# Healthcare-Robotics/assistive-gym

Measured on AMD Instinct MI355X. Metric: env_steps_per_sec, higher is better.
Workload: dtype f32; 1 GPU; FeedingJaco-v1, 4096 lockstep envs per MI355X, random-policy rollout, 5 simulation steps per env step, 50 PGS sweeps; envs_per_gpu=4096, global_envs=4096, reset_pool=256, reset=pool, parallelism=env-sharded x1, obs_allgather=False

## Files before the change

__graft_entry__.py:

```python
import os
import subprocess
import sys

ROOT = os.path.dirname(os.path.abspath(__file__))
if ROOT not in sys.path:
    sys.path.insert(0, ROOT)


def build():
    from assistive_gym_amd.build import build as build_lib
    build_lib(force=True)
    build_lib(out=os.path.join(ROOT, 'assistive_gym_amd', 'lib', 'variants', 'lvs.so'), extra=('-DAGX_PGS_LV=3',), only=['FEEDING'])
    build_lib(out=os.path.join(ROOT, 'assistive_gym_amd', 'lib', 'variants', 'scan4.so'), extra=('-DAGX_GJK_SCAN_WIDE=0', '-DAGX_GJK_SCAN_ONE=0'), only=['FEEDING'])
    build_lib(out=os.path.join(ROOT, 'assistive_gym_amd', 'lib', 'variants', 'finishgjk.so'), extra=('-DAGX_FINISH_SPILL_GJK',), only=['FEEDING'])
    build_lib(out=os.path.join(ROOT, 'assistive_gym_amd', 'lib', 'variants', 'faceplain.so'), extra=('-DAGX_FACE_PLAIN',), only=['FEEDING', 'FEEDING_M'])
    subprocess.check_call(['make', '-C', os.path.join(ROOT, 'oracle')], stdout=subprocess.DEVNULL)
    if os.path.isdir('/root/reference/assistive_gym/envs/assets'):
        from assistive_gym_amd.model import compiler
        compiler.main()
    import assistive_gym_amd
    from assistive_gym_amd import libagx
    L = libagx.load()
    missing = [e for e in libagx.EXPORTS if not hasattr(L, e)]
    assert not missing, missing


def smoke():
    import numpy as np
    sys.path.insert(0, os.path.join(ROOT, 'tests'))
    from assistive_gym_amd import libagx
    from assistive_gym_amd.blob import ModelBlob
    from assistive_gym_amd.vec_env import build_reset_pool
    from oracle_lib import Oracle
    libagx.check(libagx.load().agx_selftest(0), 'agx_selftest')
    n = 64
# ... 23 lines not shown
```

assistive_gym_amd/csrc/agx_env.h:

```cpp
#pragma once

namespace agx {

AGX_DEV void integrate(Ctx& c, const float* gvel, float dv0, float dv1) {
  float* L = c.lds; const int lane = c.lane, n = c.ndof; const float dt = c.dt;
  L[L_VEL + lane] = gvel[lane] + dv0;
  L[L_VEL + lane + 64] = gvel[lane + 64] + dv1;
  wave_sync();
  if (lane < n) {
    const int d = lane;
    float qd = L[L_VEL + d], q = L[L_ST + c.s_q + d] + dt * qd;
    if (c.hooks && (RBI(c, d, AGX_R_KIND) & 5) == 1 && !FROZEN(c, d)) {
      const float lo = DLO(c, d), hi = DHI(c, d);
      if (q < lo - AGX_LIMIT_EPS) { q = lo; qd = 0.f; } else if (q > hi + AGX_LIMIT_EPS) { q = hi; qd = 0.f; }
    }
    L[L_ST + c.s_qd + d] = qd; L[L_ST + c.s_q + d] = q;
  }
  if (lane < c.nfree) {
    const int b = lane, o = n + 6 * b; float* r = L + L_ST + c.s_free + 13 * b;
    v3 v = ld3(L + L_VEL + o), w = ld3(L + L_VEL + o + 3);
    st3(r + 7, v); st3(r + 10, w); st3(r, ld3(r) + dt * v);
    float wn = sqrtf(dot(w, w)), th = wn * dt; float dq[4];
    if (th > 1e-12f) { float sc = sinf(0.5f * th) / wn; dq[0] = w.x * sc; dq[1] = w.y * sc; dq[2] = w.z * sc; dq[3] = cosf(0.5f * th); }
    else { dq[0] = 0.5f * dt * w.x; dq[1] = 0.5f * dt * w.y; dq[2] = 0.5f * dt * w.z; dq[3] = 1.f; }
// ... 474 lines not shown
  Ctx c; ctx_init(c, blob, lds, lane);
  const int sw = c.bi[AGX_H_STATE_WORDS];
  Scratch scr = scratch_of(gscratch);
  c.E = scr.ent; c.H = scr.hdr; c.gcon = scr.con; c.dbg = gdebug;
  c.ncon = scr.meta[META_NCON]; c.nrows = scr.meta[META_NROWS]; c.first_normal = scr.meta[META_NNC]; c.nent = scr.meta[META_NENT];
  const long long t0 = gdebug ? wave_clock() : 0;
  float dv0 = 0.f, dv1 = 0.f;
  bool solved = false;
  if constexpr (LVW_COMPILED) { if (lvw_eligible(c, lds_words)) solved = pgs_lvw(c, lds, lds_words, dv0, dv1); }
  if constexpr (LVS_COMPILED) { if (!solved && lvs_eligible(c, lds_words)) { pgs_lvs(c, lds, lds_words, dv0, dv1); solved = true; } }
  if (!solved) {
    const bool rowspace = RS_MAX_ROWS > 0 && c.nrows <= RS_MAX_ROWS && c.nv <= 64 && c.nv <= RS_NVP && c.nrows > 0 && c.nent <= SOLVE_LDS_PAIRS;
    { const int np = c.nent < SOLVE_LDS_PAIRS ? c.nent : SOLVE_LDS_PAIRS;
      const f2* src = (const f2*)scr.ent; f2* dst = (f2*)(lds + L_SOLVE_ENT);
      for (int k = lane; k < np; k += 64) dst[k] = src[k]; }
    wave_sync();
    if (!(rowspace && pgs_rowspace(c, lds + L_SOLVE_ENT, dv0, dv1))) pgs(c, dv0, dv1);
  }
  warm_remember(c, scr, lane);
  const long long t1 = gdebug ? wave_clock() : 0;
  solve_tail(c, gstate, scr, sw, phase, dv0, dv1);
  if (gdebug && lane == 0) { gdebug[DBG_TIME + 5] = (float)(t1 - t0); gdebug[DBG_TIME + 6] = (float)(wave_clock() - t1); }
}

AGX_DEV void observe_dressing(const Ctx& c, float cloth_force_sum, float robot_force, float* gobs);
AGX_DEV void env_observe(const uint32_t* blob, float* gstate, float* gobs, float* lds, int lane) {
  Ctx c; ctx_init(c, blob, lds, lane);
  load_env(c, gstate, c.bi[AGX_H_STATE_WORDS]);
  kinematics(c); update_target(c);
  if constexpr (TASK == AGX_TASK_BED_BATHING) observe_bed(c, 0.f, 0.f, 0.f, gobs);
  else if constexpr (TASK == AGX_TASK_SCRATCH_ITCH) observe_scratch(c, 0.f, 0.f, 0.f, gobs);
  else if constexpr (TASK == AGX_TASK_DRESSING) observe_dressing(c, c.lds[L_ST + c.bi[AGX_H_S_TASK] + AGX_DR_FORCE_SUM], 0.f, gobs);
  else if constexpr (TASK == AGX_TASK_ARM_MANIPULATION) observe_arm(c, 0.f, 0.f, 0.f, 0.f, 0.f, gobs);
  else observe(c, 0.f, 0.f, gobs);
}

AGX_DEV float frame_speed(const Ctx& c, int link, v3 p) {
  const float* L = c.lds;
  float sv[6] = {0, 0, 0, 0, 0, 0};
  for (int d = link; d >= 0; d = RBI(c, d, AGX_R_PARENT)) { float qd = L[L_ST + c.s_qd + d]; for (int j = 0; j < 6; j++) sv[j] += L[L_S + 6 * d + j] * qd; }
  v3 xr = p - ld3(L + L_MISC + M_REF);
  v3 v = mk3(sv[3], sv[4], sv[5]) + cross(mk3(sv[0], sv[1], sv[2]), xr);
  return sqrtf(dot(v, v));
}
AGX_DEV float ee_speed_of(const Ctx& c) { return frame_speed(c, TKI(c, AGX_T_EE_LINK), ld3(c.lds + L_MISC + M_EEP)); }

// ... 629 lines not shown
```

assistive_gym_amd/csrc/agx_kernels.hip:

```cpp
#if !defined(AGX_VNAME) || !defined(AGX_KSUFFIX) || !defined(AGX_HAS_MANIFOLD)
#error "build with the -D flags of one line of agx_variants.def, see assistive_gym_amd/build.py"
#endif
#define AGX_CAT2_(a, b) a##b
#define AGX_CAT_(a, b) AGX_CAT2_(a, b)
#define AGX_K(name) AGX_CAT_(name, AGX_KSUFFIX)

#include "agx_wave.h"
#include "agx_step.h"
#include "agx_variant.h"
#if AGX_TASK == 3
#include "agx_cloth.h"
#endif

namespace {

#define AGX_BUILD_KERNEL(kernel, launcher, MF) \
extern "C" __global__ void __launch_bounds__(64, 2) \
AGX_K(kernel)(const uint32_t* __restrict__ blob, float* state, const float* actions, float* scratch, float* debug, int env0, int n_envs, int sw, int act_dim, \
              const uint8_t* __restrict__ active, int* overflow_total, float* trace, int trace_words, int phase) { \
  extern __shared__ __attribute__((aligned(16))) float lds[]; \
  const int env = env0 + blockIdx.x; \
  if (env >= n_envs || (active && !active[env])) return; \
  const int dropped = agx::env_build<MF>(blob, state + (size_t)env * sw, actions ? actions + (size_t)env * act_dim : nullptr, scratch + (size_t)env * agx::SCR_WORDS, \
                                         debug ? debug + (size_t)env * agx::DBG_WORDS : nullptr, lds, (int)threadIdx.x, \
                                         trace ? trace + (size_t)env * trace_words + (size_t)phase * 12 * (((const int*)blob)[AGX_H_NDOF] + ((const int*)blob)[AGX_H_NFREE]) : nullptr); \
  if (dropped > 0 && threadIdx.x == 0) atomicAdd(overflow_total, dropped); \
} \
void launcher(const agx_launch& L, hipStream_t st, int e0, int ne, const float* actions, float* debug, const uint8_t* active, int phase, bool trace) { \
  hipLaunchKernelGGL(AGX_K(kernel), dim3(ne), dim3(64), agx::LDS_BYTES, st, L.blob, L.state, actions, L.scratch, debug, e0, L.n_envs, L.sw, L.act_dim, active, L.overflow, \
                     trace ? L.trace : nullptr, trace ? L.trace_words : 0, phase); \
}
AGX_BUILD_KERNEL(agx_build_kernel, v_build, false)
#if AGX_HAS_MANIFOLD
AGX_BUILD_KERNEL(agx_build_mf_kernel, v_build_mf, true)
#endif
extern "C" __global__ void __launch_bounds__(64, 4)
AGX_K(agx_solve_kernel)(const uint32_t* __restrict__ blob, float* state, float* scratch, float* debug, int env0, int n_envs, int sw, const uint8_t* __restrict__ active, int phase,
                        int lds_words) {
  extern __shared__ __attribute__((aligned(16))) float lds[];
  const int env = env0 + blockIdx.x;
  if (env >= n_envs || (active && !active[env])) return;
  agx::env_solve(blob, state + (size_t)env * sw, scratch + (size_t)env * agx::SCR_WORDS, debug ? debug + (size_t)env * agx::DBG_WORDS : nullptr, lds, (int)threadIdx.x, phase,
                 lds_words);
}
extern "C" __global__ void __launch_bounds__(64, 2)
AGX_K(agx_finish_kernel)(const uint32_t* __restrict__ blob, float* state, const float* actions, float* scratch, float* obs, float* reward, uint8_t* done,
                         float* info, int env0, int n_envs, int sw, int act_dim, int obs_dim, const float* report, int report_words, float* cloth, int cloth_words) {
  extern __shared__ __attribute__((aligned(16))) float lds[];
  const int env = env0 + blockIdx.x;
  if (env >= n_envs) return;
  agx::env_finish(blob, state + (size_t)env * sw, actions + (size_t)env * act_dim, scratch + (size_t)env * agx::SCR_WORDS, obs + (size_t)env * obs_dim,
                  reward + env, done + env, info ? info + (size_t)env * AGX_INFO_COUNT : nullptr, lds, (int)threadIdx.x,
                  report ? report + (size_t)env * report_words : nullptr, cloth ? cloth + (size_t)env * cloth_words : nullptr);
}
#if AGX_TASK == 5
extern "C" __global__ void __launch_bounds__(64)
AGX_K(agx_water_kernel)(const uint32_t* __restrict__ blob, const float* __restrict__ state, const float* __restrict__ trace, float* water, float* report, int env0, int n_envs,
                        int sw, int trace_words, int cloth_words, int report_words, int nsub, const uint8_t* __restrict__ active) {
  __shared__ __attribute__((aligned(16))) float lds[agxw::LDS_WORDS];
  const int env = env0 + blockIdx.x;
  if (env >= n_envs || (active && !active[env])) return;
  agxw::water_env(blob, state + (size_t)env * sw, trace + (size_t)env * trace_words, water + (size_t)env * cloth_words, report ? report + (size_t)env * report_words : nullptr, nsub,
// ... 30 lines not shown
                         const float* __restrict__ settled, int settled_sw, const float* __restrict__ fell) {
  const int env = blockIdx.x;
  if (env >= n_envs || (mask && !mask[env])) return;
  const unsigned long long seed = seeds ? seeds[env] : seed0 + (unsigned long long)env;
  if (threadIdx.x == 0) episode[env] = 0;
  const int r = agx::env_sample(blob, state + (size_t)env * sw, (uint32_t)seed, (uint32_t)(seed >> 32), impairment_mode, gender_mode,
                                info4 ? info4 + (size_t)env * 4 : nullptr, (int)threadIdx.x, first_restart ? first_restart[env] : 0,
                                settled ? settled + (size_t)env * settled_sw : nullptr, fell ? fell + (size_t)env * sw : nullptr);
  if (chosen && threadIdx.x == 0) chosen[env] = r;
}
extern "C" __global__ void __launch_bounds__(64)
AGX_K(agx_reset_verdict_kernel)(const uint32_t* __restrict__ blob, const float* __restrict__ scratch, const uint8_t* __restrict__ active, uint8_t* work,
                                int* first_restart, const int* __restrict__ chosen, int n_envs) {
  const int env = blockIdx.x;
  if (env >= n_envs) return;
  bool again = false;
  if ((!active || active[env]) && chosen[env] >= 0) again = agx::reset_collides(blob, scratch + (size_t)env * agx::SCR_WORDS, (int)threadIdx.x);
  if (threadIdx.x == 0) { work[env] = again ? 1 : 0; if (again) first_restart[env] = chosen[env] + 1; }
}

constexpr int SWEEP_LDS_BYTES = agx::LVS_COMPILED ? agx::LVS_SOLVE_LDS_BYTES : 0;
int g_solve_lds_bytes = SWEEP_LDS_BYTES > agx::LDS_SOLVE_BYTES ? SWEEP_LDS_BYTES : agx::LDS_SOLVE_BYTES;
hipError_t v_init(void) {
  if (const char* e = getenv("AGX_SOLVE_LDS_BYTES")) { int b = atoi(e) & ~15; if (b >= agx::LDS_SOLVE_BYTES && b <= 64 * 1024) g_solve_lds_bytes = b; }
  hipError_t e = hipFuncSetAttribute((const void*)AGX_K(agx_solve_kernel), hipFuncAttributeMaxDynamicSharedMemorySize, g_solve_lds_bytes);
  if (e == hipSuccess) e = hipFuncSetAttribute((const void*)AGX_K(agx_build_kernel), hipFuncAttributeMaxDynamicSharedMemorySize, agx::LDS_BYTES);
#if AGX_HAS_MANIFOLD
  if (e == hipSuccess) e = hipFuncSetAttribute((const void*)AGX_K(agx_build_mf_kernel), hipFuncAttributeMaxDynamicSharedMemorySize, agx::LDS_BYTES);
#endif
  if (e == hipSuccess) e = hipFuncSetAttribute((const void*)AGX_K(agx_finish_kernel), hipFuncAttributeMaxDynamicSharedMemorySize, agx::LDS_BYTES);
  if (e == hipSuccess) e = hipFuncSetAttribute((const void*)AGX_K(agx_observe_kernel), hipFuncAttributeMaxDynamicSharedMemorySize, agx::LDS_BYTES);
#if AGX_TASK == 3
  if (e == hipSuccess) e = hipFuncSetAttribute((const void*)AGX_K(agx_cloth_kernel), hipFuncAttributeMaxDynamicSharedMemorySize, 160 * 1024);
#endif
  return e;
}
void v_solve(const agx_launch& L, hipStream_t st, int e0, int ne, float* debug, const uint8_t* active, int phase) {
  hipLaunchKernelGGL(AGX_K(agx_solve_kernel), dim3(ne), dim3(64), g_solve_lds_bytes, st, L.blob, L.state, L.scratch, debug, e0, L.n_envs, L.sw, active, phase, g_solve_lds_bytes / 4);
}
void v_finish(const agx_launch& L, hipStream_t st, int e0, int ne, const float* actions, float* obs, float* reward, uint8_t* done, float* info) {
  hipLaunchKernelGGL(AGX_K(agx_finish_kernel), dim3(ne), dim3(64), agx::LDS_BYTES, st, L.blob, L.state, actions, L.scratch, obs, reward, done, info, e0, L.n_envs, L.sw, L.act_dim,
                     L.obs_dim, L.report, L.report_words, L.cloth, L.cloth_words);
}
#if AGX_TASK == 5
void v_cloth(const agx_launch& L, hipStream_t st, int e0, int ne, int nsub, const uint8_t* active) {
  hipLaunchKernelGGL(AGX_K(agx_water_kernel), dim3(ne), dim3(64), 0, st, L.blob, L.state, L.trace, L.cloth, L.report, e0, L.n_envs, L.sw, L.trace_words, L.cloth_words,
                     L.report_words, nsub, active);
}
int v_cloth_lds_bytes(int nn) { (void)nn; return 4 * agxw::LDS_WORDS; }
#elif AGX_TASK == 3
void v_cloth(const agx_launch& L, hipStream_t st, int e0, int ne, int nsub, const uint8_t* active) {
  hipLaunchKernelGGL(AGX_K(agx_cloth_kernel), dim3(ne), dim3(AGX_CLOTH_THREADS), L.cloth_lds, st, L.blob, L.state, L.trace, L.cloth, L.report, e0, L.n_envs, L.sw, L.trace_words,
                     L.cloth_words, L.report_words, nsub, active);
}
int v_cloth_lds_bytes(int nn) { return 4 * agxc::lds_words(nn); }
#endif
void v_observe(const agx_launch& L, hipStream_t st, float* obs, const uint8_t* mask) {
  hipLaunchKernelGGL(AGX_K(agx_observe_kernel), dim3(L.n_envs), dim3(64), agx::LDS_BYTES, st, L.blob, L.state, obs, L.n_envs, L.sw, L.obs_dim, mask);
}
void v_sample(const agx_launch& L, hipStream_t st, const agx_sample_args& A, const uint8_t* mask, float* info4, const int* first_restart) {
  hipLaunchKernelGGL(AGX_K(agx_sample_kernel), dim3(L.n_envs), dim3(64), 0, st, L.blob, L.state, A.seed0, A.seeds, mask, A.impairment_mode, A.gender_mode, info4, L.episode, L.n_envs,
// ... 44 lines not shown
```

assistive_gym_amd/csrc/agx_pgs_lvw.h:

```cpp
#pragma once

namespace agx {

constexpr bool LVW_COMPILED = AGX_PGS_LV == 4 && LV_COMPILED;
constexpr int LVW_NG = 4;
#ifndef AGX_LVW_MAX_STEPS
#define AGX_LVW_MAX_STEPS 64
#endif
constexpr int LVW_MAX_STEPS = AGX_LVW_MAX_STEPS;
static_assert(LVW_MAX_STEPS <= 64, "lane = step");
constexpr int LVW_LIST = 64 + 4;
constexpr int LVW_DV = 0, LVW_LAM = 128, LVW_LISTS = LVW_LAM + HW_ROWS, LVW_PAIRS = LVW_LISTS + 3 * LVW_LIST;
static_assert(LVW_PAIRS % 2 == 0, "(J,B) pairs are read as 8-byte words");
static_assert(!HDR_WIDE || (HP_BASE % 2 == 0 && HQ_BASE % 4 == 0), "the compact tables are read with 8- and 4-byte loads");
static_assert(HW_DUMMY < 255, "a step list holds row indices as bytes");
constexpr uint32_t LVW_IDLE = 0x01010101u * (uint32_t)HW_DUMMY;

AGX_DEV int lvw_window(int lds_words) {
  int w = (lds_words - LVW_PAIRS) / 2;
#ifdef AGX_LV_WINDOW_CAP
  if (w > AGX_LV_WINDOW_CAP) w = AGX_LV_WINDOW_CAP;
#endif
  return w < 0 ? 0 : w;
}
AGX_DEV bool lvw_eligible(const Ctx& c, int lds_words) { return lvs_eligible(c, lds_words) && c.nv <= 96 && lds_words > LVW_PAIRS + 64 && PRM(c, AGX_P_SOLVE_WIDE) != 0.f; }

struct LvwLay { float* lds; const float* H; const float* E; int dv_addr, lam_addr, pairs_addr, far8; };

AGX_DEV int lvw_schedule(const Ctx& c, int lane, int r0, int nr, uint32_t& ss) {
  uint32_t a0 = 0u, a1 = 0u, a2 = 0u, b0 = 0u, b1 = 0u, b2 = 0u;
  if (lane < nr) { const int* Xi = (const int*)hx_row(c.H, r0 + lane); a0 = (uint32_t)Xi[H_MLO]; a1 = (uint32_t)Xi[H_MHI]; a2 = (uint32_t)Xi[H_M2]; }
  if (64 + lane < nr) { const int* Xi = (const int*)hx_row(c.H, r0 + 64 + lane); b0 = (uint32_t)Xi[H_MLO]; b1 = (uint32_t)Xi[H_MHI]; b2 = (uint32_t)Xi[H_M2]; }
  uint32_t u0 = 0u, u1 = 0u, u2 = 0u; int fill = 0; ss = LVW_IDLE;
  bool fits = true;
  auto place = [&](uint32_t m0, uint32_t m1, uint32_t m2, int r) {
    const uint64_t conflicts = wave_ballot(((u0 & m0) | (u1 & m1) | (u2 & m2)) != 0u);
    const int e = conflicts ? 64 - clz64(conflicts) : 0;
    const uint64_t room = wave_ballot(fill < LVW_NG && lane < LVW_MAX_STEPS);
    const uint64_t cand = e >= 64 ? 0ull : (room >> e) << e;
    if (!cand) fits = false;
    const int s = cand ? ffs64(cand) : -1;
    if (lane == s) { const int sh = 8 * fill; ss = (ss & ~(0xffu << sh)) | ((uint32_t)r << sh); fill++; u0 |= m0; u1 |= m1; u2 |= m2; }
  };
  const int n0 = nr < 64 ? nr : 64;
  _Pragma("nounroll") for (int r = 0; r < n0; r++) place((uint32_t)wave_bcast_i((int)a0, r), (uint32_t)wave_bcast_i((int)a1, r), (uint32_t)wave_bcast_i((int)a2, r), r0 + r);
  _Pragma("nounroll") for (int r = 64; r < nr; r++) place((uint32_t)wave_bcast_i((int)b0, r - 64), (uint32_t)wave_bcast_i((int)b1, r - 64), (uint32_t)wave_bcast_i((int)b2, r - 64), r0 + r);
  if (!fits) return -1;
  const uint64_t used = wave_ballot(fill > 0);
  return used ? 64 - clz64(used) : 0;
}
AGX_DEV int lvw_row(uint32_t ss, int j) { return (int)((ss >> (8 * j)) & 255u); }
AGX_DEV int lvw_rows4(uint32_t ss) { int m = 0; for (int j = 0; j < LVW_NG; j++) if (lvw_row(ss, j) != HW_DUMMY) m |= 1 << j; return m; }
AGX_DEV int lvw_compact(float* lds, int list, int lane, uint32_t ss, int act4) {
  uint32_t w = ss;
  for (int j = 0; j < LVW_NG; j++) if (!((act4 >> j) & 1)) w = (w & ~(0xffu << (8 * j))) | ((uint32_t)HW_DUMMY << (8 * j));
  const uint64_t m = wave_ballot(act4 != 0);
  const int n = popc64(m);
  int* L = (int*)lds + list;
  if (act4 != 0) L[wave_rank(m)] = (int)w;
  if (lane < 4) L[n + lane] = (int)LVW_IDLE;
  wave_fence();
  return n;
}

#if !defined(__HIP_DEVICE_COMPILE__) || defined(AGX_PGS_LV_CPP)
AGX_DEV void lvw_step(const LvwLay& Y, int lane, uint32_t w, bool fric) {
  const int g = lane >> 4, k = lane & (LV_G - 1), row = (int)((w >> (8 * g)) & 255u);
  const float* Q = Y.H + HQ_BASE + HQ_STRIDE * row; const int* Qi = (const int*)Q; const int* P = (const int*)(Y.H + HP_BASE + HP_STRIDE * row);
  const int off8 = P[0] & 0xffff, n = (P[0] >> 16) & 255, na = (P[0] >> 24) & 255, ab = P[1];
  const bool on = k < n;
  const int slot = 4 * k + (k < na ? (ab & 0xffff) : ((ab >> 16) & 0xffff)) - H_AB_BIAS;
  float J = 0.f, B = 0.f, v = 0.f;
  if (on) { if (off8 >= Y.far8) lv_ld2g(Y.E + (off8 >> 2) + 2 * k, J, B); else lv_ld2(Y.lds, Y.pairs_addr + off8 + 8 * k, J, B); v = lv_ld1(Y.lds, Y.dv_addr + slot); }
  const float jdv = wave_sum16(on ? J * v : 0.f);
  const float l0 = lv_ld1(Y.lds, Y.lam_addr + 4 * row);
  float lo = Q[2], hi = Q[3];
  if (fric) { hi = Q[3] * lv_ld1(Y.lds, Y.lam_addr + Qi[2]); lo = -hi; }
  const float nl = wave_clamp(l0 + (Q[1] - jdv) * Q[0], lo, hi);
  const float dl = nl - l0;
  wave_fence();
  if (on) lv_st1(Y.lds, Y.dv_addr + slot, v + B * dl);
  if (k == 0) lv_st1(Y.lds, Y.lam_addr + 4 * row, nl);
  wave_fence();
}
#else
#define LVW_SL0 "v80", "v81", "v[80:81]", "v82", "v83", "v[82:83]", "v84", "v85", "v86", "v87", "v88", "v89", "s[52:53]"
#define LVW_SL1 "v90", "v91", "v[90:91]", "v92", "v93", "v[92:93]", "v94", "v95", "v96", "v97", "v98", "v99", "s[54:55]"
#define LVW_SL2 "v100", "v101", "v[100:101]", "v102", "v103", "v[102:103]", "v104", "v105", "v106", "v107", "v108", "v109", "s[56:57]"
#define LVW_SL3 "v110", "v111", "v[110:111]", "v112", "v113", "v[112:113]", "v114", "v115", "v116", "v117", "v118", "v119", "s[58:59]"
#define LVW_QP(i) " quad_perm:[" #i "," #i "," #i "," #i "] row_mask:0xf bank_mask:0xf\n"
#define LVW_DPP(CTRL) "v_add_f32_dpp v120, v120, v120 " CTRL " row_mask:0xf bank_mask:0xf bound_ctrl:1\n"
#define LVW_S1(RID, OFF) "ds_read_u8 " RID ", %[sa] offset:" OFF "\n"
#define LVW_S1B(RID)
#define LVW_TAIL_LAST "v_add_u32_e32 %[sa], 16, %[sa]\n"
#define LVW_PRIME LVW_S1("v88", "0") LVW_S1("v98", "4") LVW_S1("v108", "8") LVW_S1("v118", "12") "s_waitcnt lgkmcnt(0)\n"
#define LVW_S2(P0, P1, PP, J, B, JB, HWA, L0, IA, LA, RID, LN, SON) \
  "v_lshl_add_u32 v126, " RID ", 4, %[hbk]\n" \
  "v_lshlrev_b32_e32 v127, 3, " RID "\n" \
  "global_load_dword " HWA ", v126, %[hq]\n" \
  "v_lshl_add_u32 " LA ", " RID ", 2, %[lamb]\n" \
  "global_load_dwordx2 " PP ", v127, %[hp]\n"
#define LVW_S3(FRIC, LBL, P0, P1, PP, J, B, JB, HWA, L0, IA, LA, RID, LN, SON) \
  "v_cmp_lt_u32_sdwa vcc, %[kreg], " P0 " src0_sel:DWORD src1_sel:BYTE_3\n" \
  "v_cmp_lt_u32_sdwa " SON ", %[kreg], " P0 " src0_sel:DWORD src1_sel:BYTE_2\n" \
  "ds_read_b32 " L0 ", " LA "\n" \
  FRIC("v_add_u32_dpp v125, " HWA ", %[lambv]" LVW_QP(2)) \
  FRIC("ds_read_b32 " LN ", v125\n") \
  "v_cndmask_b32_sdwa v124, " P1 ", " P1 ", vcc dst_sel:DWORD dst_unused:UNUSED_PAD src0_sel:WORD_1 src1_sel:WORD_0\n" \
  "v_add_u32_e32 " IA ", v124, %[k4dv]\n" \
  "v_cmp_le_u32_sdwa vcc, %[far8], " P0 " src0_sel:DWORD src1_sel:WORD_0\n" \
  "v_add_u32_sdwa v124, " P0 ", %[k8p] dst_sel:DWORD dst_unused:UNUSED_PAD src0_sel:WORD_0 src1_sel:DWORD\n" \
  "s_cbranch_vccnz " LBL "1f\n" \
  "ds_read_b64 " JB ", v124\n" \
  LBL "2:\n"
#define LVW_FAR(LBL, P0, P1, PP, J, B, JB, HWA, L0, IA, LA, RID, LN, SON) \
  LBL "1:\n" \
  "s_andn2_b64 exec, exec, vcc\n" \
  "ds_read_b64 " JB ", v124\n" \
  "s_and_b64 exec, vcc, " SON "\n" \
  "v_add_u32_sdwa v124, " P0 ", %[k8] dst_sel:DWORD dst_unused:UNUSED_PAD src0_sel:WORD_0 src1_sel:DWORD\n" \
  "global_load_dwordx2 " JB ", v124, %[E]\n" \
  "s_mov_b64 exec, -1\n" \
  "s_branch " LBL "2b\n"
// ... 11 lines not shown
#define LVW_SUBEND_LAST "s_sub_u32 s60, s60, 1\n"
#define LVW_S4(FRIC, S2TEXT_A, S2TEXT_B, S2TEXT_C, S1TEXT, S1B, TAIL, GNEXT, SUBEND, P0, P1, PP, J, B, JB, HWA, L0, IA, LA, RID, LN, SON) \
  "v_mul_f32_e32 v120, " J ", v123\n" \
  "v_cndmask_b32_e64 v120, 0, v120, " SON "\n" \
  S2TEXT_A \
  LVW_DPP("quad_perm:[1,0,3,2]") \
  S2TEXT_B \
  LVW_DPP("quad_perm:[2,3,0,1]") \
  S2TEXT_C S1TEXT \
  LVW_DPP("row_half_mirror") \
  "v_mov_b32_e32 v122, " L0 "\n" \
  TAIL \
  LVW_DPP("row_mirror") \
  S1B \
  "v_sub_f32_dpp v121, " HWA ", v120" LVW_QP(1) \
  "v_fmac_f32_dpp v122, " HWA ", v121" LVW_QP(0) \
  FRIC("v_mul_f32_dpp v121, " HWA ", " LN LVW_QP(3)) \
  FRIC("v_med3_f32 v122, v122, -v121, v121\n") \
  LVS_NOT_##FRIC("v_max_f32_dpp v121, " HWA ", v122" LVW_QP(2)) \
  LVS_NOT_##FRIC("v_min_f32_dpp v122, " HWA ", v121" LVW_QP(3)) \
  "v_sub_f32_e32 v121, v122, " L0 "\n" \
  "v_fmac_f32_e32 v123, " B ", v121\n" \
  LVW_END(LA, SON, IA, GNEXT, SUBEND)
#define LVW_S2_A(P0, P1, PP, J, B, JB, HWA, L0, IA, LA, RID, LN, SON) "v_lshl_add_u32 v126, " RID ", 4, %[hbk]\n" "v_lshlrev_b32_e32 v127, 3, " RID "\n"
#define LVW_S2_B(P0, P1, PP, J, B, JB, HWA, L0, IA, LA, RID, LN, SON) "global_load_dword " HWA ", v126, %[hq]\n" "v_lshl_add_u32 " LA ", " RID ", 2, %[lamb]\n"
#define LVW_S2_C(P0, P1, PP, J, B, JB, HWA, L0, IA, LA, RID, LN, SON) "global_load_dwordx2 " PP ", v127, %[hp]\n"
#define LVW_RID(P0, P1, PP, J, B, JB, HWA, L0, IA, LA, RID, LN, SON) RID
#define LVW_ITER(FRIC, LBL, OFF, TAIL, SUBEND, C, N1, N3) \
  "s_waitcnt vmcnt(2)\n" \
  LVS_APPLY(LVW_S3, FRIC, LBL, N1) \
  "s_waitcnt lgkmcnt(1)\n" \
  LVS_APPLY(LVW_S4, FRIC, LVS_APPLY(LVW_S2_A, N3), LVS_APPLY(LVW_S2_B, N3), LVS_APPLY(LVW_S2_C, N3), LVW_S1(LVS_APPLY(LVW_RID, C), OFF), LVW_S1B(LVS_APPLY(LVW_RID, C)), TAIL, LVS_APPLY(LVW_GATHER, N1), SUBEND, C)
#define LVW_BODY(FRIC) \
    "s_mov_b64 s[50:51], exec\n" \
    "s_mov_b64 exec, -1\n" \
    "s_mov_b32 s60, %[nst1]\n" \
     \
    LVW_PRIME \
    LVS_APPLY(LVW_S2, LVW_SL0) LVS_APPLY(LVW_S2, LVW_SL1) \
    "s_waitcnt vmcnt(2)\n" \
    LVS_APPLY(LVW_S3, FRIC, "7", LVW_SL0) \
    LVS_APPLY(LVW_GATHER, LVW_SL0) \
    LVS_APPLY(LVW_S2, LVW_SL2) \
    "8:\n" \
    LVW_ITER(FRIC, "1", "16", LVW_TAIL_STEP, LVW_SUBEND_STEP, LVW_SL0, LVW_SL1, LVW_SL3) \
    LVW_ITER(FRIC, "2", "20", LVW_TAIL_STEP, LVW_SUBEND_STEP, LVW_SL1, LVW_SL2, LVW_SL0) \
    LVW_ITER(FRIC, "3", "24", LVW_TAIL_STEP, LVW_SUBEND_STEP, LVW_SL2, LVW_SL3, LVW_SL1) \
    LVW_ITER(FRIC, "4", "28", LVW_TAIL_LAST, LVW_SUBEND_LAST, LVW_SL3, LVW_SL0, LVW_SL2) \
    "s_branch 8b\n" \
    "9:\n" \
    "s_waitcnt vmcnt(0) lgkmcnt(0)\n" \
    "s_mov_b64 exec, s[50:51]\n" \
    "s_branch 99f\n" \
    LVS_APPLY(LVW_FAR, "7", LVW_SL0) LVS_APPLY(LVW_FAR, "1", LVW_SL1) LVS_APPLY(LVW_FAR, "2", LVW_SL2) LVS_APPLY(LVW_FAR, "3", LVW_SL3) LVS_APPLY(LVW_FAR, "4", LVW_SL0) \
    "99:\n"
#define LVW_CLOBBERS \
      "v80", "v81", "v82", "v83", "v84", "v85", "v86", "v87", "v88", "v89", "v90", "v91", "v92", "v93", "v94", "v95", "v96", "v97", "v98", "v99", \
      "v100", "v101", "v102", "v103", "v104", "v105", "v106", "v107", "v108", "v109", "v110", "v111", "v112", "v113", "v114", "v115", "v116", "v117", "v118", "v119", \
      "v120", "v121", "v122", "v123", "v124", "v125", "v126", "v127", \
      "s50", "s51", "s52", "s53", "s54", "s55", "s56", "s57", "s58", "s59", "s60", "vcc", "scc", "memory"
#define LVW_ASM(FRIC) \
  asm volatile(LVW_BODY(FRIC) \
    : [sa] "+v"(sa) \
    : [nst1] "s"(nsteps - 1), [hq] "s"(Hq), [hp] "s"(Hp), [E] "s"(Y.E), [far8] "s"(Y.far8), [lamb] "s"(Y.lam_addr), [lambv] "v"(Y.lam_addr), \
      [kreg] "v"(k), [k8p] "v"(8 * k + Y.pairs_addr), [k8] "v"(8 * k), [k4dv] "v"(4 * k + Y.dv_addr - H_AB_BIAS), [hbk] "v"(4 * (lane & 3)) \
    : LVW_CLOBBERS)
AGX_DEV void lvw_part_asm(const LvwLay& Y, int lane, int list_addr, int nsteps, bool fric) {
  const int k = lane & (LV_G - 1);
  int sa = list_addr + (lane >> 4);
  const float* Hq = Y.H + HQ_BASE; const float* Hp = Y.H + HP_BASE;
  if (fric) LVW_ASM(LVS_YES); else LVW_ASM(LVS_NO);
}
#endif

AGX_DEV void lvw_part(const LvwLay& Y, int lane, int list, int nsteps, bool fric) {
  if (nsteps <= 0) return;
#if defined(__HIP_DEVICE_COMPILE__) && !defined(AGX_PGS_LV_CPP)
  lvw_part_asm(Y, lane, lv_addr(Y.lds, Y.lds + list), nsteps, fric);
#else
  for (int t = 0; t < nsteps; t++) lvw_step(Y, lane, (uint32_t)((const int*)Y.lds)[list + t], fric);
#endif
  wave_fence();
}

AGX_DEV bool pgs_lvw(Ctx& c, float* lds, int lds_words, float& dv0, float& dv1) {
  const int lane = c.lane, iters = (int)PRM(c, AGX_P_NITER);
  const int nnc = c.first_normal, nc = c.ncon, nA = nnc + nc, R = c.nrows;
  const bool two_dirs = R > nA + nc;
  uint32_t ssA, ssF;
  const int nsA = lvw_schedule(c, lane, 0, nA, ssA), nsF = nsA < 0 ? -1 : lvw_schedule(c, lane, nA, nc, ssF);
  if (nsA < 0 || nsF < 0) return false;
  LvwLay Y; Y.lds = lds; Y.H = c.H; Y.E = c.E; Y.dv_addr = lv_addr(lds, lds + LVW_DV); Y.lam_addr = lv_addr(lds, lds + LVW_LAM); Y.pairs_addr = lv_addr(lds, lds + LVW_PAIRS);
  const int LIST_FULL = LVW_LISTS, LIST_RED = LVW_LISTS + LVW_LIST, LIST_F = LVW_LISTS + 2 * LVW_LIST;
  float* LAM = lds + LVW_LAM;
  const int win = lvw_window(lds_words);
  lds[LVW_DV + lane] = 0.f; lds[LVW_DV + 64 + lane] = 0.f;
  for (int r = lane; r < HW_ROWS; r += 64) LAM[r] = 0.f;
  { const f2* src = (const f2*)c.E; f2* dst = (f2*)(lds + LVW_PAIRS); const int np = c.nent < win ? c.nent : win; for (int q = lane; q < np; q += 64) dst[q] = src[q]; }
  { int far_first = 0x2000;
    for (int r = lane; r < R; r += 64) { const int p0 = ((const int*)(c.H + HP_BASE))[HP_STRIDE * r]; const int off = (p0 & 0xffff) >> 3, n = (p0 >> 16) & 255; if (off + n > win && off < far_first) far_first = off; }
    Y.far8 = 8 * (int)wave_min((float)far_first); }
  wave_sync();
  const int rowsA4 = lane < nsA ? lvw_rows4(ssA) : 0, rowsF4 = lane < nsF ? lvw_rows4(ssF) : 0;
  const int nFull = lvw_compact(lds, LIST_FULL, lane, ssA, rowsA4);
  int nRed = 0, nF = 0, actF = -1;
  int stat_steps = 0, stat_rows = 0;
  const bool stats = c.dbg != nullptr;
  const int K = noop_period(c);
  _Pragma("nounroll") for (int it = 0; it < iters; it++) {
    const bool retest = K > 0 && it % K == 0, use = K > 0 && !retest;
    float bef[LVW_NG];
    if (retest) for (int j = 0; j < LVW_NG; j++) bef[j] = LAM[lvw_row(ssA, j)];
    lvw_part(Y, lane, use ? LIST_RED : LIST_FULL, use ? nRed : nFull, false);
    if (stats) { stat_steps += use ? nRed : nFull; const int* L = (const int*)lds + (use ? LIST_RED : LIST_FULL); const int nn = use ? nRed : nFull;
      stat_rows += wave_sum_i(lane < nn ? lvw_rows4((uint32_t)L[lane < nn ? lane : 0]) == 0 ? 0 : __builtin_popcount(lvw_rows4((uint32_t)L[lane < nn ? lane : 0])) : 0); }
// ... 5 lines not shown
    _Pragma("nounroll") for (int dir = 0; dir < (two_dirs ? 2 : 1); dir++) {
      const uint32_t ss = ssF;
      int act = 0;
      for (int j = 0; j < LVW_NG; j++) {
        const int r = lvw_row(ss, j);
        if (r != HW_DUMMY) { const float lf = LAM[r + dir * nc], ln = LAM[r - nc]; if (ln != 0.f || lf != 0.f) act |= 1 << j; }
      }
      uint32_t ssd = ss;
      if (dir) for (int j = 0; j < LVW_NG; j++) if (lvw_row(ss, j) != HW_DUMMY) ssd += (uint32_t)nc << (8 * j);
      act &= rowsF4;
      if (two_dirs || wave_any(act != actF)) { nF = lvw_compact(lds, LIST_F, lane, ssd, act); actF = act; }
      lvw_part(Y, lane, LIST_F, nF, true);
      if (stats) { stat_steps += nF; stat_rows += wave_sum_i(__builtin_popcount(act)); }
    }
  }
  wave_sync();
  dv0 = lds[LVW_DV + lane]; dv1 = lds[LVW_DV + 64 + lane];
  if (lane < nc) c.gcon[CON_STRIDE * lane + C_LAM] = LAM[nnc + lane];
  if (stats && lane == 0) { c.dbg[DBG_TIME + 16] = (float)stat_steps; c.dbg[DBG_TIME + 17] = (float)stat_rows; c.dbg[DBG_TIME + 18] = (float)(nsA + nsF); c.dbg[DBG_TIME + 19] = (float)R; }
  wave_sync();
  return true;
}

}
```

Baseline: 660,000 env-steps/s.

## Solve two environments per wave in the LVW PGS solver

Adds a paired solve path in which each 64-lane wave runs the PGS sweeps for two environments at once. Each half-wave handles one env with two row groups instead of four, and each env gets its own LDS region and global record offset. The kernel launches half as many blocks with double LDS and its launch bound drops from 4 to 3 waves. The goal is to fill lanes that sit idle when an env has only a few rows per step, at the cost of extra LDS per block, lower occupancy, and sweeps that run as long as the busier env of each pair.

```diff
diff --git a/__graft_entry__.py b/__graft_entry__.py
--- a/__graft_entry__.py
+++ b/__graft_entry__.py
@@ -11,6 +11,7 @@
     from assistive_gym_amd.build import build as build_lib
     build_lib(force=True)
     build_lib(out=os.path.join(ROOT, 'assistive_gym_amd', 'lib', 'variants', 'lvs.so'), extra=('-DAGX_PGS_LV=3',), only=['FEEDING'])
+    build_lib(out=os.path.join(ROOT, 'assistive_gym_amd', 'lib', 'variants', 'solo.so'), extra=('-DAGX_SOLVE_PAIR=0',), only=['FEEDING'])
     build_lib(out=os.path.join(ROOT, 'assistive_gym_amd', 'lib', 'variants', 'scan4.so'), extra=('-DAGX_GJK_SCAN_WIDE=0', '-DAGX_GJK_SCAN_ONE=0'), only=['FEEDING'])
     build_lib(out=os.path.join(ROOT, 'assistive_gym_amd', 'lib', 'variants', 'finishgjk.so'), extra=('-DAGX_FINISH_SPILL_GJK',), only=['FEEDING'])
     build_lib(out=os.path.join(ROOT, 'assistive_gym_amd', 'lib', 'variants', 'faceplain.so'), extra=('-DAGX_FACE_PLAIN',), only=['FEEDING', 'FEEDING_M'])
diff --git a/assistive_gym_amd/csrc/agx_env.h b/assistive_gym_amd/csrc/agx_env.h
--- a/assistive_gym_amd/csrc/agx_env.h
+++ b/assistive_gym_amd/csrc/agx_env.h
@@ -520,6 +520,33 @@
   solve_tail(c, gstate, scr, sw, phase, dv0, dv1);
   if (gdebug && lane == 0) { gdebug[DBG_TIME + 5] = (float)(t1 - t0); gdebug[DBG_TIME + 6] = (float)(wave_clock() - t1); }
 }
+#if AGX_SOLVE_PAIR
+AGX_DEV void env_solve_load(Ctx& c, Scratch& scr, const uint32_t* blob, float* gscratch, float* lds, int lane) {
+  ctx_init(c, blob, lds, lane);
+  scr = scratch_of(gscratch);
+  c.E = scr.ent; c.H = scr.hdr; c.gcon = scr.con;
+  c.ncon = scr.meta[META_NCON]; c.nrows = scr.meta[META_NROWS]; c.first_normal = scr.meta[META_NNC]; c.nent = scr.meta[META_NENT];
+}
+AGX_DEV bool env_solve_pair(const uint32_t* blob, float* gstate, float* gscratch, float* lds, int lane, int phase, int lds_words) {
+  if constexpr (!LVW_PAIRED) { (void)blob; (void)gstate; (void)gscratch; (void)lds; (void)lane; (void)phase; (void)lds_words; return false; }
+  else {
+    { Ctx c0, c1; Scratch s0, s1;
+      env_solve_load(c0, s0, blob, gscratch, lds, lane); env_solve_load(c1, s1, blob, gscratch + SCR_WORDS, lds + lds_words, lane);
+      if (!lvw_eligible(c0, lds_words) || !lvw_eligible(c1, lds_words)) return false;
+      if (!pgs_lvw_pair(c0, c1, lds, lds_words)) return false; }
+    _Pragma("nounroll") for (int e = 0; e < 2; e++) {
+      Ctx c; Scratch scr;
+      env_solve_load(c, scr, blob, gscratch + (size_t)e * SCR_WORDS, lds + e * lds_words, lane);
+      const int sw = c.bi[AGX_H_STATE_WORDS];
+      float dv0, dv1;
+      lvw_pair_result(c, c.lds, dv0, dv1);
+      warm_remember(c, scr, lane);
+      solve_tail(c, gstate + (size_t)e * sw, scr, sw, phase, dv0, dv1);
+    }
+    return true;
+  }
+}
+#endif
 
 AGX_DEV void observe_dressing(const Ctx& c, float cloth_force_sum, float robot_force, float* gobs);
 AGX_DEV void env_observe(const uint32_t* blob, float* gstate, float* gobs, float* lds, int lane) {
diff --git a/assistive_gym_amd/csrc/agx_kernels.hip b/assistive_gym_amd/csrc/agx_kernels.hip
--- a/assistive_gym_amd/csrc/agx_kernels.hip
+++ b/assistive_gym_amd/csrc/agx_kernels.hip
@@ -34,10 +34,42 @@
 #if AGX_HAS_MANIFOLD
 AGX_BUILD_KERNEL(agx_build_mf_kernel, v_build_mf, true)
 #endif
-extern "C" __global__ void __launch_bounds__(64, 4)
+#if AGX_SOLVE_PAIR && AGX_PGS_LV == 4 && AGX_MAX_DOF <= 16 && AGX_MAX_BLOCK <= 10 && AGX_TASK == 0
+#define AGX_SOLVE_PAIRED 1
+#define AGX_SOLVE_END_PARAM , int env_end
+#define AGX_SOLVE_END_ARG(x) , x
+#else
+#define AGX_SOLVE_PAIRED 0
+#define AGX_SOLVE_END_PARAM
+#define AGX_SOLVE_END_ARG(x)
+#endif
+constexpr bool SOLVE_PAIRED = agx::LVW_PAIRED;
+static_assert(SOLVE_PAIRED == (AGX_SOLVE_PAIRED != 0), "the preprocessor's statement of agx::LVW_PAIRED");
+#ifndef AGX_SOLVE_WAVES
+#define AGX_SOLVE_WAVES (SOLVE_PAIRED ? 3 : 4)
+#endif
+extern "C" __global__ void __launch_bounds__(64, AGX_SOLVE_WAVES)
 AGX_K(agx_solve_kernel)(const uint32_t* __restrict__ blob, float* state, float* scratch, float* debug, int env0, int n_envs, int sw, const uint8_t* __restrict__ active, int phase,
-                        int lds_words) {
-  extern __shared__ __attribute__((aligned(16))) float lds[];
+                        int lds_words AGX_SOLVE_END_PARAM) {
+  extern __shared__ __attribute__((aligned(16))) float lds[];
+#if AGX_SOLVE_PAIRED
+  {
+    const bool pair = debug == nullptr;
+    const int envA = wave_uniform(env0 + (pair ? 2 : 1) * (int)blockIdx.x);
+    if (env_end > n_envs) env_end = n_envs;
+    const bool has0 = envA < env_end && (!active || active[envA]), has1 = pair && envA + 1 < env_end && (!active || active[envA + 1]);
+    int lane2 = (int)threadIdx.x;
+    asm volatile("" : "+v"(lane2));
+    if (has0 && has1 && agx::env_solve_pair(blob, state + (size_t)envA * sw, scratch + (size_t)envA * agx::SCR_WORDS, lds, lane2, phase, lds_words)) return;
+    _Pragma("nounroll") for (int e = 0; e < 2; e++) {
+      const int lane = (int)threadIdx.x;
+      if (e ? has1 : has0) agx::env_solve(blob, state + (size_t)(envA + e) * sw, scratch + (size_t)(envA + e) * agx::SCR_WORDS, debug ? debug + (size_t)(envA + e) * agx::DBG_WORDS : nullptr,
+                                          lds, lane, phase, lds_words);
+      wave_sync();
+    }
+    return;
+  }
+#endif
   const int env = env0 + blockIdx.x;
   if (env >= n_envs || (active && !active[env])) return;
   agx::env_solve(blob, state + (size_t)env * sw, scratch + (size_t)env * agx::SCR_WORDS, debug ? debug + (size_t)env * agx::DBG_WORDS : nullptr, lds, (int)threadIdx.x, phase,
@@ -114,8 +146,8 @@
 constexpr int SWEEP_LDS_BYTES = agx::LVS_COMPILED ? agx::LVS_SOLVE_LDS_BYTES : 0;
 int g_solve_lds_bytes = SWEEP_LDS_BYTES > agx::LDS_SOLVE_BYTES ? SWEEP_LDS_BYTES : agx::LDS_SOLVE_BYTES;
 hipError_t v_init(void) {
-  if (const char* e = getenv("AGX_SOLVE_LDS_BYTES")) { int b = atoi(e) & ~15; if (b >= agx::LDS_SOLVE_BYTES && b <= 64 * 1024) g_solve_lds_bytes = b; }
-  hipError_t e = hipFuncSetAttribute((const void*)AGX_K(agx_solve_kernel), hipFuncAttributeMaxDynamicSharedMemorySize, g_solve_lds_bytes);
+  if (const char* e = getenv("AGX_SOLVE_LDS_BYTES")) { int b = atoi(e) & ~15; if (b >= agx::LDS_SOLVE_BYTES && b <= (SOLVE_PAIRED ? 32 : 64) * 1024) g_solve_lds_bytes = b; }
+  hipError_t e = hipFuncSetAttribute((const void*)AGX_K(agx_solve_kernel), hipFuncAttributeMaxDynamicSharedMemorySize, (SOLVE_PAIRED ? 2 : 1) * g_solve_lds_bytes);
   if (e == hipSuccess) e = hipFuncSetAttribute((const void*)AGX_K(agx_build_kernel), hipFuncAttributeMaxDynamicSharedMemorySize, agx::LDS_BYTES);
 #if AGX_HAS_MANIFOLD
   if (e == hipSuccess) e = hipFuncSetAttribute((const void*)AGX_K(agx_build_mf_kernel), hipFuncAttributeMaxDynamicSharedMemorySize, agx::LDS_BYTES);
@@ -128,7 +160,9 @@
   return e;
 }
 void v_solve(const agx_launch& L, hipStream_t st, int e0, int ne, float* debug, const uint8_t* active, int phase) {
-  hipLaunchKernelGGL(AGX_K(agx_solve_kernel), dim3(ne), dim3(64), g_solve_lds_bytes, st, L.blob, L.state, L.scratch, debug, e0, L.n_envs, L.sw, active, phase, g_solve_lds_bytes / 4);
+  const bool pair = SOLVE_PAIRED && !debug;
+  hipLaunchKernelGGL(AGX_K(agx_solve_kernel), dim3(pair ? (ne + 1) / 2 : ne), dim3(64), (SOLVE_PAIRED ? 2 : 1) * g_solve_lds_bytes, st, L.blob, L.state, L.scratch, debug, e0, L.n_envs, L.sw,
+                     active, phase, g_solve_lds_bytes / 4 AGX_SOLVE_END_ARG(e0 + ne));
 }
 void v_finish(const agx_launch& L, hipStream_t st, int e0, int ne, const float* actions, float* obs, float* reward, uint8_t* done, float* info) {
   hipLaunchKernelGGL(AGX_K(agx_finish_kernel), dim3(ne), dim3(64), agx::LDS_BYTES, st, L.blob, L.state, actions, L.scratch, obs, reward, done, info, e0, L.n_envs, L.sw, L.act_dim,
diff --git a/assistive_gym_amd/csrc/agx_pgs_lvw.h b/assistive_gym_amd/csrc/agx_pgs_lvw.h
--- a/assistive_gym_amd/csrc/agx_pgs_lvw.h
+++ b/assistive_gym_amd/csrc/agx_pgs_lvw.h
@@ -4,6 +4,11 @@
 
 constexpr bool LVW_COMPILED = AGX_PGS_LV == 4 && LV_COMPILED;
 constexpr int LVW_NG = 4;
+#ifndef AGX_SOLVE_PAIR
+#define AGX_SOLVE_PAIR 1
+#endif
+constexpr bool LVW_PAIRED = AGX_SOLVE_PAIR != 0 && LVW_COMPILED;
+constexpr int LVW_NG_PAIR = 2;
 #ifndef AGX_LVW_MAX_STEPS
 #define AGX_LVW_MAX_STEPS 64
 #endif
@@ -25,9 +30,9 @@
 }
 AGX_DEV bool lvw_eligible(const Ctx& c, int lds_words) { return lvs_eligible(c, lds_words) && c.nv <= 96 && lds_words > LVW_PAIRS + 64 && PRM(c, AGX_P_SOLVE_WIDE) != 0.f; }
 
-struct LvwLay { float* lds; const float* H; const float* E; int dv_addr, lam_addr, pairs_addr, far8; };
-
-AGX_DEV int lvw_schedule(const Ctx& c, int lane, int r0, int nr, uint32_t& ss) {
+struct LvwLay { float* lds; const float* H; const float* E; int dv_addr, lam_addr, pairs_addr, far8, rec; };
+
+AGX_DEV int lvw_schedule(const Ctx& c, int lane, int r0, int nr, uint32_t& ss, int ng = LVW_NG) {
   uint32_t a0 = 0u, a1 = 0u, a2 = 0u, b0 = 0u, b1 = 0u, b2 = 0u;
   if (lane < nr) { const int* Xi = (const int*)hx_row(c.H, r0 + lane); a0 = (uint32_t)Xi[H_MLO]; a1 = (uint32_t)Xi[H_MHI]; a2 = (uint32_t)Xi[H_M2]; }
   if (64 + lane < nr) { const int* Xi = (const int*)hx_row(c.H, r0 + 64 + lane); b0 = (uint32_t)Xi[H_MLO]; b1 = (uint32_t)Xi[H_MHI]; b2 = (uint32_t)Xi[H_M2]; }
@@ -36,7 +41,7 @@
   auto place = [&](uint32_t m0, uint32_t m1, uint32_t m2, int r) {
     const uint64_t conflicts = wave_ballot(((u0 & m0) | (u1 & m1) | (u2 & m2)) != 0u);
     const int e = conflicts ? 64 - clz64(conflicts) : 0;
-    const uint64_t room = wave_ballot(fill < LVW_NG && lane < LVW_MAX_STEPS);
+    const uint64_t room = wave_ballot(fill < ng && lane < LVW_MAX_STEPS);
     const uint64_t cand = e >= 64 ? 0ull : (room >> e) << e;
     if (!cand) fits = false;
     const int s = cand ? ffs64(cand) : -1;
@@ -66,12 +71,13 @@
 #if !defined(__HIP_DEVICE_COMPILE__) || defined(AGX_PGS_LV_CPP)
 AGX_DEV void lvw_step(const LvwLay& Y, int lane, uint32_t w, bool fric) {
   const int g = lane >> 4, k = lane & (LV_G - 1), row = (int)((w >> (8 * g)) & 255u);
-  const float* Q = Y.H + HQ_BASE + HQ_STRIDE * row; const int* Qi = (const int*)Q; const int* P = (const int*)(Y.H + HP_BASE + HP_STRIDE * row);
+  const float* H = Y.H + (Y.rec >> 2); const float* E = Y.E + (Y.rec >> 2);
+  const float* Q = H + HQ_BASE + HQ_STRIDE * row; const int* Qi = (const int*)Q; const int* P = (const int*)(H + HP_BASE + HP_STRIDE * row);
   const int off8 = P[0] & 0xffff, n = (P[0] >> 16) & 255, na = (P[0] >> 24) & 255, ab = P[1];
   const bool on = k < n;
   const int slot = 4 * k + (k < na ? (ab & 0xffff) : ((ab >> 16) & 0xffff)) - H_AB_BIAS;
   float J = 0.f, B = 0.f, v = 0.f;
-  if (on) { if (off8 >= Y.far8) lv_ld2g(Y.E + (off8 >> 2) + 2 * k, J, B); else lv_ld2(Y.lds, Y.pairs_addr + off8 + 8 * k, J, B); v = lv_ld1(Y.lds, Y.dv_addr + slot); }
+  if (on) { if (off8 >= Y.far8) lv_ld2g(E + (off8 >> 2) + 2 * k, J, B); else lv_ld2(Y.lds, Y.pairs_addr + off8 + 8 * k, J, B); v = lv_ld1(Y.lds, Y.dv_addr + slot); }
   const float jdv = wave_sum16(on ? J * v : 0.f);
   const float l0 = lv_ld1(Y.lds, Y.lam_addr + 4 * row);
   float lo = Q[2], hi = Q[3];
@@ -94,11 +100,20 @@
 #define LVW_S1B(RID)
 #define LVW_TAIL_LAST "v_add_u32_e32 %[sa], 16, %[sa]\n"
 #define LVW_PRIME LVW_S1("v88", "0") LVW_S1("v98", "4") LVW_S1("v108", "8") LVW_S1("v118", "12") "s_waitcnt lgkmcnt(0)\n"
+#if AGX_SOLVE_PAIR
+#define LVW_PADDR(RID) "v_lshl_add_u32 v127, " RID ", 3, %[pbk]\n"
+#define LVW_LAMB "%[lambv]"
+#define LVW_FAR8_C "v"
+#else
+#define LVW_PADDR(RID) "v_lshlrev_b32_e32 v127, 3, " RID "\n"
+#define LVW_LAMB "%[lamb]"
+#define LVW_FAR8_C "s"
+#endif
 #define LVW_S2(P0, P1, PP, J, B, JB, HWA, L0, IA, LA, RID, LN, SON) \
   "v_lshl_add_u32 v126, " RID ", 4, %[hbk]\n" \
-  "v_lshlrev_b32_e32 v127, 3, " RID "\n" \
+  LVW_PADDR(RID) \
   "global_load_dword " HWA ", v126, %[hq]\n" \
-  "v_lshl_add_u32 " LA ", " RID ", 2, %[lamb]\n" \
+  "v_lshl_add_u32 " LA ", " RID ", 2, " LVW_LAMB "\n" \
   "global_load_dwordx2 " PP ", v127, %[hp]\n"
 #define LVW_S3(FRIC, LBL, P0, P1, PP, J, B, JB, HWA, L0, IA, LA, RID, LN, SON) \
   "v_cmp_lt_u32_sdwa vcc, %[kreg], " P0 " src0_sel:DWORD src1_sel:BYTE_3\n" \
@@ -156,8 +171,8 @@
   "v_sub_f32_e32 v121, v122, " L0 "\n" \
   "v_fmac_f32_e32 v123, " B ", v121\n" \
   LVW_END(LA, SON, IA, GNEXT, SUBEND)
-#define LVW_S2_A(P0, P1, PP, J, B, JB, HWA, L0, IA, LA, RID, LN, SON) "v_lshl_add_u32 v126, " RID ", 4, %[hbk]\n" "v_lshlrev_b32_e32 v127, 3, " RID "\n"
-#define LVW_S2_B(P0, P1, PP, J, B, JB, HWA, L0, IA, LA, RID, LN, SON) "global_load_dword " HWA ", v126, %[hq]\n" "v_lshl_add_u32 " LA ", " RID ", 2, %[lamb]\n"
+#define LVW_S2_A(P0, P1, PP, J, B, JB, HWA, L0, IA, LA, RID, LN, SON) "v_lshl_add_u32 v126, " RID ", 4, %[hbk]\n" LVW_PADDR(RID)
+#define LVW_S2_B(P0, P1, PP, J, B, JB, HWA, L0, IA, LA, RID, LN, SON) "global_load_dword " HWA ", v126, %[hq]\n" "v_lshl_add_u32 " LA ", " RID ", 2, " LVW_LAMB "\n"
 #define LVW_S2_C(P0, P1, PP, J, B, JB, HWA, L0, IA, LA, RID, LN, SON) "global_load_dwordx2 " PP ", v127, %[hp]\n"
 #define LVW_RID(P0, P1, PP, J, B, JB, HWA, L0, IA, LA, RID, LN, SON) RID
 #define LVW_ITER(FRIC, LBL, OFF, TAIL, SUBEND, C, N1, N3) \
@@ -193,11 +208,18 @@
       "v100", "v101", "v102", "v103", "v104", "v105", "v106", "v107", "v108", "v109", "v110", "v111", "v112", "v113", "v114", "v115", "v116", "v117", "v118", "v119", \
       "v120", "v121", "v122", "v123", "v124", "v125", "v126", "v127", \
       "s50", "s51", "s52", "s53", "s54", "s55", "s56", "s57", "s58", "s59", "s60", "vcc", "scc", "memory"
+#if AGX_SOLVE_PAIR
+#define LVW_ASM_LAMB
+#define LVW_ASM_PBK , [pbk] "v"(Y.rec)
+#else
+#define LVW_ASM_LAMB [lamb] "s"(Y.lam_addr),
+#define LVW_ASM_PBK
+#endif
 #define LVW_ASM(FRIC) \
   asm volatile(LVW_BODY(FRIC) \
     : [sa] "+v"(sa) \
-    : [nst1] "s"(nsteps - 1), [hq] "s"(Hq), [hp] "s"(Hp), [E] "s"(Y.E), [far8] "s"(Y.far8), [lamb] "s"(Y.lam_addr), [lambv] "v"(Y.lam_addr), \
-      [kreg] "v"(k), [k8p] "v"(8 * k + Y.pairs_addr), [k8] "v"(8 * k), [k4dv] "v"(4 * k + Y.dv_addr - H_AB_BIAS), [hbk] "v"(4 * (lane & 3)) \
+    : [nst1] "s"(nsteps - 1), [hq] "s"(Hq), [hp] "s"(Hp), [E] "s"(Y.E), [far8] LVW_FAR8_C(Y.far8), LVW_ASM_LAMB [lambv] "v"(Y.lam_addr), \
+      [kreg] "v"(k), [k8p] "v"(8 * k + Y.pairs_addr), [k8] "v"(8 * k + Y.rec), [k4dv] "v"(4 * k + Y.dv_addr - H_AB_BIAS), [hbk] "v"(4 * (lane & 3) + Y.rec) LVW_ASM_PBK \
     : LVW_CLOBBERS)
 AGX_DEV void lvw_part_asm(const LvwLay& Y, int lane, int list_addr, int nsteps, bool fric) {
   const int k = lane & (LV_G - 1);
@@ -224,7 +246,7 @@
   uint32_t ssA, ssF;
   const int nsA = lvw_schedule(c, lane, 0, nA, ssA), nsF = nsA < 0 ? -1 : lvw_schedule(c, lane, nA, nc, ssF);
   if (nsA < 0 || nsF < 0) return false;
-  LvwLay Y; Y.lds = lds; Y.H = c.H; Y.E = c.E; Y.dv_addr = lv_addr(lds, lds + LVW_DV); Y.lam_addr = lv_addr(lds, lds + LVW_LAM); Y.pairs_addr = lv_addr(lds, lds + LVW_PAIRS);
+  LvwLay Y; Y.lds = lds; Y.H = c.H; Y.E = c.E; Y.rec = 0; Y.dv_addr = lv_addr(lds, lds + LVW_DV); Y.lam_addr = lv_addr(lds, lds + LVW_LAM); Y.pairs_addr = lv_addr(lds, lds + LVW_PAIRS);
   const int LIST_FULL = LVW_LISTS, LIST_RED = LVW_LISTS + LVW_LIST, LIST_F = LVW_LISTS + 2 * LVW_LIST;
   float* LAM = lds + LVW_LAM;
   const int win = lvw_window(lds_words);
@@ -276,4 +298,91 @@
   return true;
 }
 
-}
+#if AGX_SOLVE_PAIR
+struct LvwSide { uint32_t ssA, ssF; int rowsA4, rowsF4, nc, nFull, nRed, nF, actF; float* LAM; };
+AGX_DEV int lvw_compact2(float* lds0, int list, int lane, int side, uint32_t ss, int act2) {
+  typedef unsigned short __attribute__((may_alias)) u16a;
+  uint32_t w = ss & 0xffffu;
+  for (int j = 0; j < LVW_NG_PAIR; j++) if (!((act2 >> j) & 1)) w = (w & ~(0xffu << (8 * j))) | ((uint32_t)HW_DUMMY << (8 * j));
+  const uint64_t m = wave_ballot(act2 != 0);
+  const int n = popc64(m);
+  u16a* L = (u16a*)((int*)lds0 + list) + side;
+  for (int t = lane; t < LVW_LIST; t += 64) if (t >= n) L[2 * t] = (unsigned short)(LVW_IDLE & 0xffffu);
+  if (act2 != 0) L[2 * wave_rank(m)] = (unsigned short)w;
+  wave_fence();
+  return n;
+}
+AGX_DEV bool lvw_pair_prepare(const Ctx& c, float* lds0, float* lds, int lds_words, int side, LvwSide& S, LvwLay& Y) {
+  const int lane = c.lane;
+  const int nnc = c.first_normal, nc = c.ncon, nA = nnc + nc, R = c.nrows;
+  const int nsA = lvw_schedule(c, lane, 0, nA, S.ssA, LVW_NG_PAIR), nsF = nsA < 0 ? -1 : lvw_schedule(c, lane, nA, nc, S.ssF, LVW_NG_PAIR);
+  if (nsA < 0 || nsF < 0) return false;
+  S.nc = nc; S.LAM = lds + LVW_LAM; S.nRed = 0; S.nF = 0; S.actF = -1;
+  Y.lds = lds0; Y.rec = side * 4 * SCR_WORDS;
+  Y.dv_addr = lv_addr(lds0, lds + LVW_DV); Y.lam_addr = lv_addr(lds0, lds + LVW_LAM); Y.pairs_addr = lv_addr(lds0, lds + LVW_PAIRS);
+  const int win = lvw_window(lds_words);
+  lds[LVW_DV + lane] = 0.f; lds[LVW_DV + 64 + lane] = 0.f;
+  for (int r = lane; r < HW_ROWS; r += 64) S.LAM[r] = 0.f;
+  { const f2* src = (const f2*)c.E; f2* dst = (f2*)(lds + LVW_PAIRS); const int np = c.nent < win ? c.nent : win; for (int q = lane; q < np; q += 64) dst[q] = src[q]; }
+  { int far_first = 0x2000;
+    for (int r = lane; r < R; r += 64) { const int p0 = ((const int*)(c.H + HP_BASE))[HP_STRIDE * r]; const int off = (p0 & 0xffff) >> 3, n = (p0 >> 16) & 255; if (off + n > win && off < far_first) far_first = off; }
+    Y.far8 = 8 * (int)wave_min((float)far_first); }
+  S.rowsA4 = lane < nsA ? lvw_rows4(S.ssA) : 0; S.rowsF4 = lane < nsF ? lvw_rows4(S.ssF) : 0;
+  return true;
+}
+AGX_DEV bool pgs_lvw_pair(const Ctx& c0, const Ctx& c1, float* lds0, int lds_words) {
+  const int lane = c0.lane, iters = (int)PRM(c0, AGX_P_NITER);
+  float* const lds1 = lds0 + lds_words;
+  LvwSide S[2]; LvwLay Ys[2];
+  if (!lvw_pair_prepare(c0, lds0, lds0, lds_words, 0, S[0], Ys[0])) return false;
+  if (!lvw_pair_prepare(c1, lds0, lds1, lds_words, 1, S[1], Ys[1])) return false;
+  const bool e = lane >= 32;
+  LvwLay Y; Y.lds = lds0; Y.H = c0.H; Y.E = c0.E;
+  Y.dv_addr = e ? Ys[1].dv_addr : Ys[0].dv_addr; Y.lam_addr = e ? Ys[1].lam_addr : Ys[0].lam_addr; Y.pairs_addr = e ? Ys[1].pairs_addr : Ys[0].pairs_addr;
+  Y.far8 = e ? Ys[1].far8 : Ys[0].far8; Y.rec = e ? Ys[1].rec : Ys[0].rec;
+  const int LIST_FULL = LVW_LISTS, LIST_RED = LVW_LISTS + LVW_LIST, LIST_F = LVW_LISTS + 2 * LVW_LIST;
+  const bool two_dirs = c0.nrows > c0.first_normal + 2 * c0.ncon || c1.nrows > c1.first_normal + 2 * c1.ncon;
+  wave_sync();
+  _Pragma("unroll") for (int s = 0; s < 2; s++) S[s].nFull = lvw_compact2(lds0, LIST_FULL, lane, s, S[s].ssA, S[s].rowsA4);
+  const int K0 = noop_period(c0), K1 = noop_period(c1), K = K0 > K1 ? K0 : K1;
+  const bool rule[2] = {K0 > 0, K1 > 0};
+  if (K > 0) _Pragma("unroll") for (int s = 0; s < 2; s++) if (!rule[s]) S[s].nRed = lvw_compact2(lds0, LIST_RED, lane, s, S[s].ssA, S[s].rowsA4);
+  _Pragma("nounroll") for (int it = 0; it < iters; it++) {
+    const bool retest = K > 0 && it % K == 0, use = K > 0 && !retest;
+    float bef[2][LVW_NG_PAIR];
+    if (retest) _Pragma("unroll") for (int s = 0; s < 2; s++) if (rule[s]) for (int j = 0; j < LVW_NG_PAIR; j++) bef[s][j] = S[s].LAM[lvw_row(S[s].ssA, j)];
+    { const int n0 = use ? S[0].nRed : S[0].nFull, n1 = use ? S[1].nRed : S[1].nFull;
+      lvw_part(Y, lane, use ? LIST_RED : LIST_FULL, n0 > n1 ? n0 : n1, false); }
+    if (retest) _Pragma("unroll") for (int s = 0; s < 2; s++) if (rule[s]) {
+      int act = 0;
+      for (int j = 0; j < LVW_NG_PAIR; j++) if (S[s].LAM[lvw_row(S[s].ssA, j)] != bef[s][j]) act |= 1 << j;
+      S[s].nRed = lvw_compact2(lds0, LIST_RED, lane, s, S[s].ssA, act & S[s].rowsA4);
+    }
+    _Pragma("nounroll") for (int dir = 0; dir < (two_dirs ? 2 : 1); dir++) {
+      _Pragma("unroll") for (int s = 0; s < 2; s++) {
+        const uint32_t ss = S[s].ssF; const int nc = S[s].nc;
+        int act = 0;
+        for (int j = 0; j < LVW_NG_PAIR; j++) {
+          const int r = lvw_row(ss, j);
+          if (r != HW_DUMMY) { const float lf = S[s].LAM[r + dir * nc], ln = S[s].LAM[r - nc]; if (ln != 0.f || lf != 0.f) act |= 1 << j; }
+        }
+        uint32_t ssd = ss;
+        if (dir) for (int j = 0; j < LVW_NG_PAIR; j++) if (lvw_row(ss, j) != HW_DUMMY) ssd += (uint32_t)nc << (8 * j);
+        act &= S[s].rowsF4;
+        if (two_dirs || wave_any(act != S[s].actF)) { S[s].nF = lvw_compact2(lds0, LIST_F, lane, s, ssd, act); S[s].actF = act; }
+      }
+      lvw_part(Y, lane, LIST_F, S[0].nF > S[1].nF ? S[0].nF : S[1].nF, true);
+    }
+  }
+  wave_sync();
+  return true;
+}
+AGX_DEV void lvw_pair_result(Ctx& c, const float* lds, float& dv0, float& dv1) {
+  const int lane = c.lane;
+  dv0 = lds[LVW_DV + lane]; dv1 = lds[LVW_DV + 64 + lane];
+  if (lane < c.ncon) c.gcon[CON_STRIDE * lane + C_LAM] = lds[LVW_LAM + c.first_normal + lane];
+  wave_sync();
+}
+#endif
+
+}
```

Measured after the change: 679,400 env-steps/s, median of 6. 2.9% higher.
